# bjo5029/causal-vae

Hardware: AMD Instinct MI355X
Metric: training samples/sec on 128^3 vessel volumes (3D CausalVAE train step) (higher is better)
Workload: dtype bf16; 1 GPU; 3D vessel CausalVAE train step, 128^3 bf16 volumes (z-scored N(0,1)), batch 4/GPU, Adam lr 0.0001, ELBO = MSE-sum + 2000*MSE-sum(m) + KLD; global_batch=4, per_gpu_batch=4, parallelism=dp1, params=15346957

## Files before the change

### causal_vae_amd/csrc/conv_mfma.hip

```cpp
#include "common.h"

#ifdef CVAE_STAMP
#define CVAE_STAMP_SLOTS 32
#define CVAE_STAMP_WGS 8192
__device__ unsigned long long g_stamp[(size_t)CVAE_STAMP_WGS * CVAE_STAMP_SLOTS];
#define STAMP(i)                                                                                                         \
    do {                                                                                                                 \
        if (t == 0 && stamp_wg < CVAE_STAMP_WGS) g_stamp[(size_t)stamp_wg * CVAE_STAMP_SLOTS + (i)] = __builtin_readcyclecounter(); \
    } while (0)
#else
#define STAMP(i)
#endif

namespace {

CVAE_TUNABLE(BD_GS, 8);
CVAE_TUNABLE(APIPE, 3);
CVAE_TUNABLE(UPFULL_MIN_GRID, 2048);
CVAE_TUNABLE(UPFULL_MIN_WG, 512);
CVAE_TUNABLE(XPAIR_MIN_WGS, 2048);
CVAE_TUNABLE(XPAIR_2D_MIN_WGS, 512);
CVAE_TUNABLE(WG_TILES, 16);
CVAE_TUNABLE(WG_MIN_WG, 64);

// ... 1037 lines not shown
    float amx = 0.f;
    for (int64_t i = (((int64_t)blockIdx.x - tb.blk_start[ti]) * 256 + threadIdx.x) * 4; i < n; i += (int64_t)nb * 1024) {
        float v[4];
#pragma unroll
        for (int u = 0; u < 4; ++u) {
            const int64_t iu = i + u;
            const int e = (int)(iu % CH);
            int64_t rr = iu / CH;
            int cs, cl, tap;
            if (!for_up) { cs = (int)(rr % Cs); rr /= Cs; const int ch = (int)(rr % (Cl / CH)); tap = (int)(rr / (Cl / CH)); cl = ch * CH + e; }
            else { cl = (int)(rr % Cl); rr /= Cl; const int ch = (int)(rr % (Cs / CH)); tap = (int)(rr / (Cs / CH)); cs = ch * CH + e; }
            v[u] = w[((int64_t)cs * Cl + cl) * taps + tap];
            amx = fmaxf(amx, fabsf(v[u]));
            v[u] = __builtin_amdgcn_fmed3f(v[u] * mul, -CVAE_FP8_MAX, CVAE_FP8_MAX);
        }
        int c = __builtin_amdgcn_cvt_pk_fp8_f32(v[0], v[1], 0, false);
        c = __builtin_amdgcn_cvt_pk_fp8_f32(v[2], v[3], c, true);
        *(int*)(out + i) = c;
    }
    __shared__ float red[4];
    if (tb.amax[ti]) amax_publish_wg(tb.amax[ti], amx, blockIdx.x, red);
}

#define F8LAYER_MAX 16
struct F8LayerIdx { int in[F8LAYER_MAX], w[F8LAYER_MAX], out[F8LAYER_MAX]; int count; };
__global__ __launch_bounds__(1024) void fp8_scale_update_kernel(unsigned* __restrict__ amax, float* __restrict__ scale, float* __restrict__ inv_scale, int n, float headroom,
                                                                F8LayerIdx li, float* __restrict__ dscale, unsigned* __restrict__ ticket) {
    static_assert(CVAE_AMAX_SLOTS == 4096, "one uint4 per thread");
    __shared__ float red[16];
    __shared__ unsigned last;
    const int t = threadIdx.x, lane = t & 63, wave = t >> 6, i = blockIdx.x;
    uint4* a4 = (uint4*)amax + (size_t)i * (CVAE_AMAX_SLOTS / 4);
    const uint4 v = a4[t];
    a4[t] = make_uint4(0u, 0u, 0u, 0u);
    float a = fmaxf(fmaxf(__uint_as_float(v.x), __uint_as_float(v.y)), fmaxf(__uint_as_float(v.z), __uint_as_float(v.w)));
#pragma unroll
    for (int o = 32; o > 0; o >>= 1) a = fmaxf(a, __shfl_xor(a, o, 64));
    if (lane == 0) red[wave] = a;
    __syncthreads();
    if (t == 0) {
        float m = 0.f;
        for (int w_ = 0; w_ < 16; ++w_) m = fmaxf(m, red[w_]);
        if (m > 0.f) {
            const float s_ = headroom * m / CVAE_FP8_MAX;
            __hip_atomic_store(scale + i, s_, __ATOMIC_RELAXED, __HIP_MEMORY_SCOPE_AGENT);
            __hip_atomic_store(inv_scale + i, 1.f / s_, __ATOMIC_RELAXED, __HIP_MEMORY_SCOPE_AGENT);
        }
        asm volatile("s_waitcnt vmcnt(0)" ::: "memory");
        const unsigned got = __hip_atomic_fetch_add(ticket, 1u, __ATOMIC_RELAXED, __HIP_MEMORY_SCOPE_AGENT);
        last = (got == (unsigned)n - 1u) ? 1u : 0u;
    }
    __syncthreads();
    if (last && li.count > 0) {
        if (t < li.count) {
            const float si = __hip_atomic_load(scale + li.in[t], __ATOMIC_RELAXED, __HIP_MEMORY_SCOPE_AGENT);
            const float sw = __hip_atomic_load(scale + li.w[t], __ATOMIC_RELAXED, __HIP_MEMORY_SCOPE_AGENT);
            dscale[2 * t] = si * sw;
            dscale[2 * t + 1] = li.out[t] >= 0 ? 1.f / __hip_atomic_load(scale + li.out[t], __ATOMIC_RELAXED, __HIP_MEMORY_SCOPE_AGENT) : 0.f;
        }
    }
    if (last && t == 0) __hip_atomic_store(ticket, 0u, __ATOMIC_RELAXED, __HIP_MEMORY_SCOPE_AGENT);
}

__global__ __launch_bounds__(256) void absmax_kernel(const void* __restrict__ src, int dtype, int64_t n, unsigned* __restrict__ slots) {
    float amx = 0.f;
    for (int64_t i = blockIdx.x * (int64_t)blockDim.x + threadIdx.x; i < n; i += (int64_t)gridDim.x * blockDim.x)
        amx = fmaxf(amx, fabsf(dtype == CVAE_BF16 ? to_f32(((const bf16*)src)[i]) : ((const float*)src)[i]));
    __shared__ float red[4];
    amax_publish_wg(slots, amx, blockIdx.x, red);
}

#define PAIR_MAX 16
struct PairTable {
    const float* w[PAIR_MAX];
    void* down[PAIR_MAX];
    void* up[PAIR_MAX];
    int Cs[PAIR_MAX], Cl[PAIR_MAX], blk_start[PAIR_MAX + 1];
    int count;
    int f8dir[PAIR_MAX];
    fp8* f8out[PAIR_MAX];
    const float* inv_scale[PAIR_MAX];
    unsigned* amax[PAIR_MAX];
};
template <typename T, int TAPS>
__global__ __launch_bounds__(256) void pack_weight_pairs_kernel(PairTable tb) {
    constexpr int TT = 16, TSPLIT = TAPS / TT, TP = TT + 1;
    __shared__ float tile[16 * 17 * TP];
    int ti = 0;
    while (ti + 1 < tb.count && (int)blockIdx.x >= tb.blk_start[ti + 1]) ++ti;
    const int Cs = tb.Cs[ti], Cl = tb.Cl[ti];
    int blk = (int)blockIdx.x - tb.blk_start[ti];
    const int tq = blk % TSPLIT; blk /= TSPLIT;
    const int nclt = Cl / 16, ncst = Cs / 16;
    const int cst = blk / nclt, clt = blk % nclt, cs0 = cst * 16, cl0 = clt * 16;
    const float* w = tb.w[ti];
    const int f8dir = tb.f8dir[ti];
    float amx = 0.f;
#pragma unroll
    for (int it = 0; it < 4; ++it) {
        const int i = threadIdx.x + it * 256, f = i & 3, cl = (i >> 2) & 15, cs = i >> 6;
        const float4 v = *(const float4*)(w + ((size_t)(cs0 + cs) * Cl + cl0 + cl) * TAPS + tq * TT + 4 * f);
        float* d = tile + (cs * 17 + cl) * TP + 4 * f;
        d[0] = v.x; d[1] = v.y; d[2] = v.z; d[3] = v.w;
        amx = fmaxf(fmaxf(amx, fmaxf(fabsf(v.x), fabsf(v.y))), fmaxf(fabsf(v.z), fabsf(v.w)));
    }
    __syncthreads();
    T* od = (T*)tb.down[ti];
    T* ou = (T*)tb.up[ti];
    const float mul8 = f8dir ? tb.inv_scale[ti][0] : 1.f;
    const int tg = threadIdx.x >> 5, e0 = (threadIdx.x & 31) * 8, a = e0 >> 4, b0 = e0 & 15;
#pragma unroll
    for (int tl = tg; tl < TT; tl += 8) {
        const int tap = tq * TT + tl;
        __attribute__((aligned(16))) T vd[8], vu[8];
#pragma unroll
        for (int q = 0; q < 8; ++q) {
            vd[q] = from_f32<T>(tile[(a * 17 + b0 + q) * TP + tl]);
            vu[q] = from_f32<T>(tile[((b0 + q) * 17 + a) * TP + tl]);
        }
        T* pd = od + ((size_t)(tap * nclt + clt) * Cs + cs0 + a) * 16 + b0;
        T* pu = ou + ((size_t)(tap * ncst + cst) * Cl + cl0 + a) * 16 + b0;
        constexpr int NU = (8 * sizeof(T)) / 16;
        if (f8dir != 1) {
#pragma unroll
            for (int u = 0; u < NU; ++u) ((uint4*)pd)[u] = ((const uint4*)vd)[u];
        }
        if (f8dir != 2) {
#pragma unroll
            for (int u = 0; u < NU; ++u) ((uint4*)pu)[u] = ((const uint4*)vu)[u];
        }
        if (f8dir) {
            float v8[8];
#pragma unroll
            for (int q = 0; q < 8; ++q) v8[q] = f8dir == 1 ? tile[(a * 17 + b0 + q) * TP + tl] : tile[((b0 + q) * 17 + a) * TP + tl];
            fp8* p8 = f8dir == 1 ? tb.f8out[ti] + ((size_t)(tap * (Cl / 32) + (cl0 >> 5)) * Cs + cs0 + a) * 32 + (cl0 & 16) + b0
                                 : tb.f8out[ti] + ((size_t)(tap * (Cs / 32) + (cs0 >> 5)) * Cl + cl0 + a) * 32 + (cs0 & 16) + b0;
            *(uint2*)p8 = pack8_fp8(v8, mul8);
        }
    }
    if (f8dir && tb.amax[ti]) {
        __syncthreads();
        amax_publish_wg(tb.amax[ti], amx, blockIdx.x, tile);
    }
}

#define WG_MULTI_MAX 8
struct WgradEntry {
    const void* S; const void* L; float* ws; float* bias_ws;
    ConvGeom g;
    int n_split, cb, tg, bias_mode;
    int xb;
};
struct WgradTable { WgradEntry e[WG_MULTI_MAX]; int blk_start[WG_MULTI_MAX + 1]; int count; };

template <typename T, int ND>
__global__ __launch_bounds__(512, sizeof(T) == 2 ? 4 : 2) void conv_wgrad_kernel(WgradTable tb) {
    int ti = 0;
    while (ti + 1 < tb.count && (int)blockIdx.x >= tb.blk_start[ti + 1]) ++ti;
    const T* __restrict__ S = (const T*)tb.e[ti].S;
    const T* __restrict__ L = (const T*)tb.e[ti].L;
    float* __restrict__ ws = tb.e[ti].ws;
    float* __restrict__ bias_ws = tb.e[ti].bias_ws;
    const ConvGeom g = tb.e[ti].g;
    const int n_split = tb.e[ti].n_split, bias_mode = tb.e[ti].bias_mode, grid_y = tb.e[ti].cb;
    const int xb = (ND == 2) ? tb.e[ti].xb : 0;
    int lb = (int)blockIdx.x - tb.blk_start[ti];
    const int bx = lb % n_split; lb /= n_split;
    const int by = lb % grid_y, bz = lb / grid_y;
    using TL = Tile<ND, 128>;
    constexpr int NT = 512;
    constexpr int TD = TL::TD, TH = TL::TH, TW = TL::TW;
    constexpr int IW1 = 2 * TW + 2, IW = IW1 + (ND == 2 ? 2 : 0), IH = 2 * TH + 2;
    constexpr int SROW = 64 * sizeof(T), LROW = 32 * sizeof(T);
    constexpr int S_BYTES = 128 * SROW;
    constexpr int FB = 8 * sizeof(T);
    extern __shared__ __attribute__((aligned(16))) char smem[];
    char* s_lds = smem;
    char* l_lds = smem + S_BYTES;
    const int t = threadIdx.x, lane = t & 63, wave = t >> 6;
    const int cl_blocks = g.Cl / 32;
    const int cs0 = (by / cl_blocks) * 64, cl0 = (by % cl_blocks) * 32;
    const int kd = (ND == 3) ? bz : 0;
    const int kh = wave & 3, sg = wave >> 2;
    constexpr int LHALF = IW / 2, LPLANE = TD * IH * LHALF;
    auto s_byte = [](int m, int c) -> int { return m * SROW + ((((c >> 3) ^ (((m >> 1) & 1) << 2)) << 3) + (c & 7)) * (int)sizeof(T); };
    auto l_row = [](int line, int x) -> int { return (x & 1) * LPLANE + line * LHALF + (x >> 1); };
    const int tiles_per_b = g.tiles_d * g.tiles_h * g.tiles_w, total_tiles = (xb ? (g.B + 1) / 2 : g.B) * tiles_per_b;
#ifdef CVAE_STAMP
    const unsigned stamp_wg = blockIdx.x;
    if (t == 0 && stamp_wg < CVAE_STAMP_WGS) {
        g_stamp[(size_t)stamp_wg * CVAE_STAMP_SLOTS + 30] = wall_clock64();
        g_stamp[(size_t)stamp_wg * CVAE_STAMP_SLOTS + 29] = ((unsigned long long)__builtin_amdgcn_s_getreg(63508) << 32) | __builtin_amdgcn_s_getreg(63492);
    }
    int stamp_it = 0;
#endif
    STAMP(0);

    f32x16 acc[4];
#pragma unroll
    for (int k = 0; k < 4; ++k)
#pragma unroll
        for (int e = 0; e < 16; ++e) acc[k][e] = 0.f;

    const bool bias_s = bias_mode == 1 && (by % cl_blocks) == 0 && kd == 0;
    const bool bias_l = bias_mode == 2 && (by / cl_blocks) == 0 && (ND == 2 || kd == 1 || kd == 2);
    float bacc = 0.f;
    constexpr int SN = (128 * 8) / NT, LNPOS = TD * IH * IW, LN = (LNPOS * 4 + NT - 1) / NT;
    Piece<T> sp[SN], lp[LN];
    unsigned okmask = 0;
    const int s_sample = g.sd * g.sh * g.sw * g.Cs, l_sample = g.ld * g.lh * g.lw * g.Cl;
    auto load_tile = [&](int tile) {
        int tt = tile;
        const int tw_i = tt % g.tiles_w; tt /= g.tiles_w;
        const int th_i = tt % g.tiles_h; tt /= g.tiles_h;
        const int td_i = tt % g.tiles_d;
        const int b = (tt / g.tiles_d) * (1 + xb);
        const int o0d = td_i * TD, o0h = th_i * TH, o0w = tw_i * TW;
        const T* Sb = S + (size_t)b * s_sample + cs0;
        const T* Lb = L + (size_t)b * l_sample + cl0;
        const bool b1ok = b + 1 < g.B;
        okmask = 0;
        int tz = t;
        asm volatile("" : "+v"(tz));
#pragma unroll
        for (int i = 0; i < SN; ++i) {
            const int it = tz + i * NT, piece = it & 7, m = it >> 3;
            const int w = m % TW, hh = m / TW % TH, d = m / (TW * TH);
            const int sx = (xb && w >= TW / 2) ? 1 : 0;
            const int od = o0d + d, oh = o0h + hh, ow = o0w + w - sx * (TW / 2);
            const bool ok = (od < g.sd) & (oh < g.sh) & (ow < g.sw) & (!sx | b1ok);
            const unsigned off = ((min(od, g.sd - 1) * g.sh + min(oh, g.sh - 1)) * g.sw + min(ow, g.sw - 1)) * g.Cs + piece * 8 + ((sx && b1ok) ? (unsigned)s_sample : 0u);
            piece_load_raw<T>(sp[i], Sb + off);
            okmask |= (unsigned)ok << i;
        }
#pragma unroll
        for (int i = 0; i < LN; ++i) {
            const int it = tz + i * NT, piece = it & 3, pos = min(it >> 2, LNPOS - 1);
            const int x = pos % IW, y = pos / IW % IH, d = pos / (IW * IH);
            const int sx = (xb && x >= IW / 2) ? 1 : 0;
            const int lz = (ND == 3) ? 2 * (o0d + d) - 1 + kd : 0, ly = 2 * o0h - 1 + y, lx = 2 * o0w - 1 + x - sx * (IW / 2);
            const bool ok = (lz >= 0) & (lz < g.ld) & (ly >= 0) & (ly < g.lh) & (lx >= 0) & (lx < g.lw) & (!sx | b1ok) & (xb | (x < IW1));
            const unsigned off = ((min(max(lz, 0), g.ld - 1) * g.lh + min(max(ly, 0), g.lh - 1)) * g.lw + min(max(lx, 0), g.lw - 1)) * g.Cl + piece * 8 + ((sx && b1ok) ? (unsigned)l_sample : 0u);
            piece_load_raw<T>(lp[i], Lb + off);
            okmask |= (unsigned)ok << (SN + i);
        }
    };
    if (bx < total_tiles) load_tile(bx);
    for (int tile = bx; tile < total_tiles; tile += n_split) {
        __syncthreads();
#ifdef CVAE_STAMP
        if (stamp_it < 8) STAMP(2 + 3 * stamp_it);
#endif
        {
            int tz = t;
            asm volatile("" : "+v"(tz));
#pragma unroll
            for (int i = 0; i < SN; ++i) {
                const int it = tz + i * NT;
                piece_store_sel<T>(sp[i], (okmask >> i) & 1, s_lds + s_byte(it >> 3, (it & 7) * 8));
            }
#pragma unroll
            for (int i = 0; i < LN; ++i) {
                const int it = tz + i * NT, pos = it >> 2;
                if (it < LNPOS * 4) piece_store_sel<T>(lp[i], (okmask >> (SN + i)) & 1, l_lds + (l_row(pos / IW, pos % IW) * 4 + (it & 3)) * FB);
            }
        }
        __syncthreads();
#ifdef CVAE_STAMP
        if (stamp_it < 8) STAMP(3 + 3 * stamp_it);
#endif
        if (tile + n_split < total_tiles) load_tile(tile + n_split);
        if (bias_s) {
            const int c = t & 63, pg = t >> 6;
#pragma unroll 4
            for (int j = 0; j < 16; ++j) bacc += to_f32(*(const T*)(s_lds + s_byte(pg * 16 + j, c)));
        } else if (bias_l) {
            const int c = t & 31, pg = t >> 5;
#pragma unroll 4
            for (int j = 0; j < 32; ++j) {
                const int pp = pg + 16 * j;
                const int xx = pp % (2 * TW), yy = pp / (2 * TW) % (2 * TH), dd = pp / (4 * TW * TH);
                const int xs = xx + 1 + ((xb && xx >= TW) ? 2 : 0);
                bacc += to_f32(*(const T*)(l_lds + l_row(dd * IH + yy + 1, xs) * LROW + c * (int)sizeof(T)));
            }
        }
        if constexpr (sizeof(T) == 2) {
            const int gq = lane >> 4, i16 = lane & 15, q = i16 >> 2, p = i16 & 3;
            const int hk = gq >> 1, colblk = gq & 1;
            typedef __attribute__((address_space(3))) bf16x4 lds_bf16x4;
            const char* abase[2];
            const char* bbase[2];
#pragma unroll
            for (int jj = 0; jj < 2; ++jj) {
                const int r0 = 8 * hk + 4 * jj + q;
                abase[jj] = s_lds + s_byte(r0, sg * 32 + 16 * colblk + 4 * p);
                bbase[jj] = l_lds + l_row(2 * (r0 / TW) + kh, 2 * (r0 % TW) + ((xb && (r0 % TW) >= TW / 2) ? 2 : 0)) * LROW + (16 * colblk + 4 * p) * 2;
            }
#pragma unroll
            for (int c = 0; c < 8; ++c) {
                const int hh_c = (16 * c / TW) % TH, d_c = (16 * c) / (TW * TH);
                bf16x8 a;
#pragma unroll
                for (int jj = 0; jj < 2; ++jj) {
                    const bf16x4 v = __builtin_amdgcn_ds_read_tr16_b64_v4bf16((lds_bf16x4*)(abase[jj] + 16 * c * SROW));
                    a[4 * jj + 0] = v[0]; a[4 * jj + 1] = v[1]; a[4 * jj + 2] = v[2]; a[4 * jj + 3] = v[3];
                }
#pragma unroll
                for (int kw = 0; kw < 4; ++kw) {
                    bf16x8 bv;
#pragma unroll
                    for (int jj = 0; jj < 2; ++jj) {
                        const char* bp = bbase[jj] + (((kw & 1) * LPLANE + (d_c * IH + 2 * hh_c) * LHALF + (kw >> 1)) * LROW);
                        const bf16x4 v = __builtin_amdgcn_ds_read_tr16_b64_v4bf16((lds_bf16x4*)bp);
                        bv[4 * jj + 0] = v[0]; bv[4 * jj + 1] = v[1]; bv[4 * jj + 2] = v[2]; bv[4 * jj + 3] = v[3];
                    }
                    acc[kw] = __builtin_amdgcn_mfma_f32_32x32x16_bf16(a, bv, acc[kw], 0, 0, 0);
                }
            }
        } else {
            const int r = lane & 31, hk = lane >> 5;
#pragma unroll 1
            for (int mm = 0; mm < 128; mm += 2) {
                const int m = mm + hk;
                const int w = m % TW, hh = m / TW % TH, d = m / (TW * TH);
                const int line = d * IH + 2 * hh + kh;
                const float a = *(const float*)(s_lds + s_byte(m, sg * 32 + r));
#pragma unroll
                for (int kw = 0; kw < 4; ++kw) {
                    const float bv = *(const float*)(l_lds + l_row(line, 2 * w + kw + ((xb && w >= TW / 2) ? 2 : 0)) * LROW + r * 4);
                    acc[kw] = __builtin_amdgcn_mfma_f32_32x32x2f32(a, bv, acc[kw], 0, 0, 0);
                }
            }
        }
#ifdef CVAE_STAMP
        if (stamp_it < 8) STAMP(4 + 3 * stamp_it);
        ++stamp_it;
#endif
    }
    STAMP(26);
    if (bias_s || bias_l) {
        __syncthreads();
        float* red = (float*)s_lds;
        red[t] = bacc;
        __syncthreads();
        if (bias_s && t < 64) {
            float v = 0.f;
#pragma unroll
            for (int q = 0; q < 8; ++q) v += red[q * 64 + t];
            bias_ws[((size_t)(by / cl_blocks) * n_split + bx) * 64 + t] = v;
        }
        if (bias_l && t < 32) {
            float v = 0.f;
#pragma unroll
            for (int q = 0; q < 16; ++q) v += red[q * 32 + t];
            const int half = (ND == 3) ? kd - 1 : 0, nhalf = (ND == 3) ? 2 : 1;
            bias_ws[(((size_t)(by % cl_blocks) * nhalf + half) * n_split + bx) * 32 + t] = v;
        }
    }
    const int col = lane & 31, hq = lane >> 5;
    float* slab = ws + ((size_t)(bz * grid_y + by) * n_split + bx) * 32768;
#pragma unroll
    for (int e = 0; e < 16; ++e) {
        const int row = sg * 32 + (e & 3) + 8 * (e >> 2) + 4 * hq;
        *(float4*)(slab + ((kh * 64 + row) * 32 + col) * 4) = make_float4(acc[0][e], acc[1][e], acc[2][e], acc[3][e]);
    }
#ifdef CVAE_STAMP
    __builtin_amdgcn_s_waitcnt(0);
    STAMP(27);
    if (t == 0 && stamp_wg < CVAE_STAMP_WGS) g_stamp[(size_t)stamp_wg * CVAE_STAMP_SLOTS + 31] = wall_clock64();
#endif
}

struct WgradReduceEntry {
    const float* ws; float* dW; const float* bias_ws; float* dbias;
    int Cs, Cl, n_split, cb, dw_blocks, bias_n, bias_rows, bias_width;
};
struct WgradReduceTable { WgradReduceEntry e[WG_MULTI_MAX]; int blk_start[WG_MULTI_MAX + 1]; int count, taps; };
__global__ __launch_bounds__(256) void wgrad_reduce_kernel(WgradReduceTable tb) {
    int ti = 0;
    while (ti + 1 < tb.count && (int)blockIdx.x >= tb.blk_start[ti + 1]) ++ti;
    const float* __restrict__ ws = tb.e[ti].ws;
    float* __restrict__ dW = tb.e[ti].dW;
    const float* __restrict__ bias_ws = tb.e[ti].bias_ws;
    float* __restrict__ dbias = tb.e[ti].dbias;
    const int Cl = tb.e[ti].Cl, taps = tb.taps, n_split = tb.e[ti].n_split, cb = tb.e[ti].cb, dw_blocks = tb.e[ti].dw_blocks;
    const int bias_n = tb.e[ti].bias_n, bias_rows = tb.e[ti].bias_rows, bias_width = tb.e[ti].bias_width;
    const int lbx = (int)blockIdx.x - tb.blk_start[ti];
    __shared__ float4 part[4][64];
    if (lbx >= dw_blocks) {
        __shared__ float bred[4][64];
        const int ch = (lbx - dw_blocks) * 64 + (threadIdx.x & 63), q = threadIdx.x >> 6;
        float v = 0.f;
        if (ch < bias_n) {
            const float* base = bias_ws + (size_t)(ch / bias_width) * bias_rows * bias_width + (ch % bias_width);
            for (int r = q; r < bias_rows; r += 4) v += base[(size_t)r * bias_width];
        }
        bred[q][threadIdx.x & 63] = v;
        __syncthreads();
        if (q == 0 && ch < bias_n) dbias[ch] = bred[0][threadIdx.x] + bred[1][threadIdx.x] + bred[2][threadIdx.x] + bred[3][threadIdx.x];
        return;
    }
    const int cl_blocks = Cl / 32;
    int bi = lbx;
    const int rowpair = bi % 32; bi /= 32;
    const int kh = bi % 4; bi /= 4;
    const int grp = bi;
    const int kd = grp / cb, blk = grp % cb;
    const int lane64 = threadIdx.x & 63, q = threadIdx.x >> 6;
    const int row = rowpair * 2 + (lane64 >> 5), col = lane64 & 31;
    const float* base = ws + (size_t)grp * n_split * 32768 + ((kh * 64 + row) * 32 + col) * 4;
    float4 a = make_float4(0.f, 0.f, 0.f, 0.f);
    constexpr int U = 8;
    for (int x0 = q; x0 < n_split; x0 += 4 * U) {
        float4 v[U];
#pragma unroll
        for (int u = 0; u < U; ++u) v[u] = *(const float4*)(base + (size_t)min(x0 + 4 * u, n_split - 1) * 32768);
#pragma unroll
        for (int u = 0; u < U; ++u)
            if (x0 + 4 * u < n_split) { a.x += v[u].x; a.y += v[u].y; a.z += v[u].z; a.w += v[u].w; }
    }
    part[q][lane64] = a;
    __syncthreads();
    if (q == 0) {
        const float4 b = part[1][lane64], c = part[2][lane64], d = part[3][lane64];
        a.x += b.x + c.x + d.x; a.y += b.y + c.y + d.y; a.z += b.z + c.z + d.z; a.w += b.w + c.w + d.w;
        const int cs = (blk / cl_blocks) * 64 + row, cl = (blk % cl_blocks) * 32 + col;
        *(float4*)(dW + ((size_t)cs * Cl + cl) * taps + kd * 16 + kh * 4) = a;
    }
}

#define WGRAD_MAX_WG 512
template <typename T, int ND> constexpr size_t wgrad_lds_bytes() {
    using TL = Tile<ND, 128>;
    return (size_t)128 * 64 * sizeof(T) + (size_t)TL::TD * (2 * TL::TH + 2) * (2 * TL::TW + 2 + (ND == 2 ? 2 : 0)) * 32 * sizeof(T);
}
template <typename T, int ND>
int plan_wgrad(const void* S, const void* L, float* ws, float* dW, float* dbias, int bias_mode, ConvGeom g, WgradEntry* me, WgradReduceEntry* re, int* main_blocks,
               int* reduce_blocks, long long n_split_req = 0) {
    using TL = Tile<ND, 128>;
    g.tiles_d = (g.sd + TL::TD - 1) / TL::TD; g.tiles_h = (g.sh + TL::TH - 1) / TL::TH; g.tiles_w = (g.sw + TL::TW - 1) / TL::TW;
    const int xb = (ND == 2 && g.sw <= TL::TW / 2 && g.B >= 2) ? 1 : 0;
    const long long total_tiles = (long long)(xb ? (g.B + 1) / 2 : g.B) * g.tiles_d * g.tiles_h * g.tiles_w;
    const int cb = (g.Cs / 64) * (g.Cl / 32), tg = (ND == 3) ? 4 : 1;
    long long n_split = WGRAD_MAX_WG / ((long long)cb * tg);
    long long floor_split = 256 / ((long long)cb * tg);
    if (floor_split > total_tiles) floor_split = total_tiles;
    long long by_tiles = total_tiles / 4;
    if (by_tiles < floor_split) by_tiles = floor_split;
    if (n_split > by_tiles) n_split = by_tiles;
    {
        long long req = (total_tiles + WG_TILES - 1) / WG_TILES;
        const long long groups = (long long)cb * tg;
        if (req * groups < WG_MIN_WG) req = (WG_MIN_WG + groups - 1) / groups;
        if (req < n_split) n_split = req;
    }
    if (n_split_req > 0 && n_split_req < n_split) n_split = n_split_req;
    if (n_split < 1) n_split = 1;
    if (n_split > total_tiles) n_split = total_tiles;
    if ((long long)cb * tg * n_split > (1 << 24)) return CVAE_E_BADSHAPE;
    const long long wgs = (long long)cb * tg * n_split;
    float* bias_ws = ws + (size_t)(wgs > WGRAD_MAX_WG ? wgs : WGRAD_MAX_WG) * 32768;
    if (!dbias) bias_mode = 0;
    *me = WgradEntry{S, L, ws, bias_ws, g, (int)n_split, cb, tg, bias_mode, xb};
    *main_blocks = (int)wgs;
    const int dw_blocks = cb * tg * 4 * 32;
    const int bias_n = bias_mode == 1 ? g.Cs : (bias_mode == 2 ? g.Cl : 0), bias_width = bias_mode == 1 ? 64 : 32;
    const int bias_rows = (int)n_split * ((bias_mode == 2 && ND == 3) ? 2 : 1);
    *re = WgradReduceEntry{ws, dW, bias_ws, dbias, g.Cs, g.Cl, (int)n_split, cb, dw_blocks, bias_n, bias_rows, bias_width};
    *reduce_blocks = dw_blocks + (bias_n + 63) / 64;
    return CVAE_OK;
}
template <typename T, int ND>
int launch_wgrad_tables(WgradTable& mt, WgradReduceTable& rt, hipStream_t stream) {
    constexpr size_t LDS = wgrad_lds_bytes<T, ND>();
    static_assert(LDS <= 160 * 1024, "LDS tile exceeds the 160 KiB of a CDNA4 CU");
    auto kern = conv_wgrad_kernel<T, ND>;
    static bool attr_set = false;
    if (!attr_set) {
        if (hipFuncSetAttribute((const void*)kern, hipFuncAttributeMaxDynamicSharedMemorySize, (int)LDS) != hipSuccess) return CVAE_E_LAUNCH;
        attr_set = true;
    }
    rt.taps = (ND == 3) ? 64 : 16;
    hipLaunchKernelGGL(kern, dim3((unsigned)mt.blk_start[mt.count]), dim3(512), LDS, stream, mt);
    CVAE_CHECK_LAUNCH();
    hipLaunchKernelGGL(wgrad_reduce_kernel, dim3((unsigned)rt.blk_start[rt.count]), dim3(256), 0, stream, rt);
    CVAE_CHECK_LAUNCH();
    return CVAE_OK;
}
template <typename T, int ND>
int launch_wgrad(const void* S, const void* L, float* ws, float* dW, float* dbias, int bias_mode, ConvGeom g, hipStream_t stream) {
    WgradTable mt;
    WgradReduceTable rt;
    int mb, rb;
    const int rc = plan_wgrad<T, ND>(S, L, ws, dW, dbias, bias_mode, g, &mt.e[0], &rt.e[0], &mb, &rb);
    if (rc != CVAE_OK) return rc;
    mt.count = rt.count = 1;
    mt.blk_start[0] = rt.blk_start[0] = 0;
    mt.blk_start[1] = mb; rt.blk_start[1] = rb;
    return launch_wgrad_tables<T, ND>(mt, rt, stream);
}

bool geom_ok(int64_t B, int64_t sd, int64_t sh, int64_t sw, int64_t Cs, int64_t ld, int64_t lh, int64_t lw, int64_t Cl, int nd) {
    if (nd != 2 && nd != 3) return false;
    if (B < 0 || sd <= 0 || sh <= 0 || sw <= 0 || Cs <= 0 || ld <= 0 || lh <= 0 || lw <= 0 || Cl <= 0) return false;
    if (B > 65535 || sd > 32767 || sh > 32767 || sw > 32767 || ld > 65535 || lh > 65535 || lw > 65535) return false;
    if (nd == 2 && (sd != 1 || ld != 1)) return false;
    if (sd * sh * sw * Cs >= (int64_t(1) << 31) || ld * lh * lw * Cl >= (int64_t(1) << 31)) return false;
    auto pair_ok = [](int64_t s, int64_t l) { return s == l / 2; };
    if (nd == 3 && !pair_ok(sd, ld)) return false;
    return pair_ok(sh, lh) && pair_ok(sw, lw) && lh >= 2 && lw >= 2 && (nd == 2 || ld >= 2);
}

}

int cvae_conv_down_c1(const void* L, int l_dtype, const float* w, const float* bias, const void* mask, void* S, int64_t B, int64_t sd, int64_t sh, int64_t sw,
                      int64_t Cs, int64_t ld, int64_t lh, int64_t lw, int nd, int dtype, int act, hipStream_t stream, F8Side f8 = F8Side{nullptr, nullptr, nullptr});
int cvae_conv_up_c1(const void* S, const float* w, const float* bias, const void* mask, void* L, int64_t B, int64_t sd, int64_t sh, int64_t sw,
                    int64_t Cs, int64_t ld, int64_t lh, int64_t lw, int nd, int dtype, int act, hipStream_t stream, long long walk_units = 0);
int cvae_conv_up_c1_fp8in_impl(const void* S8, const float* w, const float* bias, void* L, float in_scale, int64_t B, int64_t sd, int64_t sh, int64_t sw, int64_t Cs, int act,
                               hipStream_t stream);
size_t cvae_conv_wgrad_c1_workspace_bytes(int64_t Cs, int nd);
int cvae_conv_wgrad_c1(const void* S, const void* L, int l_dtype, float* dW, float* dbias, float* dbias_l, void* workspace, size_t workspace_bytes, int64_t B, int64_t sd, int64_t sh,
                       int64_t sw, int64_t Cs, int64_t ld, int64_t lh, int64_t lw, int nd, int dtype, hipStream_t stream);

#ifdef CVAE_STAMP
extern "C" int cvae_debug_stamps(unsigned long long* host, size_t count) {
    if (count > (size_t)CVAE_STAMP_WGS * CVAE_STAMP_SLOTS) return CVAE_E_BADSHAPE;
    return hipMemcpyFromSymbol(host, HIP_SYMBOL(g_stamp), count * sizeof(unsigned long long)) == hipSuccess ? CVAE_OK : CVAE_E_LAUNCH;
}
#endif

extern "C" int cvae_conv_pack_weight(const float* w, void* packed, int64_t Cs, int64_t Cl, int nd, int for_up, int dtype, void* stream) {
    if ((nd != 2 && nd != 3) || Cs <= 0 || Cl <= 0) return CVAE_E_BADSHAPE;
    if ((!for_up && Cl % 16) || (for_up && (Cs % 16 || Cl % 32))) return CVAE_E_UNSUPPORTED;
    if (!w || !packed) return CVAE_E_NULLPTR;
    const int taps = (nd == 3) ? 64 : 16;
    const int64_t n = Cs * Cl * taps;
    if (dtype == CVAE_BF16) hipLaunchKernelGGL(pack_weight_kernel<bf16>, dim3(cvae_grid_1d(n, 256)), dim3(256), 0, (hipStream_t)stream, w, (bf16*)packed, (int)Cs, (int)Cl, taps, for_up);
    else if (dtype == CVAE_F32) hipLaunchKernelGGL(pack_weight_kernel<float>, dim3(cvae_grid_1d(n, 256)), dim3(256), 0, (hipStream_t)stream, w, (float*)packed, (int)Cs, (int)Cl, taps, for_up);
    else return CVAE_E_DTYPE;
    CVAE_CHECK_LAUNCH();
    return CVAE_OK;
}

static bool fp8_pack_ok(int64_t Cs, int64_t Cl, int for_up) { return for_up ? (Cs % 32 == 0 && Cl % 32 == 0 && Cl > 1) : (Cl % 32 == 0 && Cs % 64 == 0); }
extern "C" int cvae_conv_pack_weight_pairs(const float* const* w, void* const* packed_down, void* const* packed_up, const int64_t* Cs, const int64_t* Cl,
                                           const int* f8dir, void* const* f8out, const float* const* inv_scale_dev, void* const* amax_slots,
                                           int count, int nd, int dtype, void* stream) {
    if ((nd != 2 && nd != 3) || count < 0) return CVAE_E_BADSHAPE;
    if (count == 0) return CVAE_OK;
    if (!w || !packed_down || !packed_up || !Cs || !Cl) return CVAE_E_NULLPTR;
    if (dtype != CVAE_BF16 && dtype != CVAE_F32) return CVAE_E_DTYPE;
    const int tsplit = (nd == 3) ? 4 : 1;
    for (int c0 = 0; c0 < count; c0 += PAIR_MAX) {
        PairTable tb;
        const int cnt = (count - c0 < PAIR_MAX) ? count - c0 : PAIR_MAX;
        long long blocks = 0;
        for (int i = 0; i < cnt; ++i) {
            const int64_t cs = Cs[c0 + i], cl = Cl[c0 + i];
            if (cs <= 0 || cl <= 0) return CVAE_E_BADSHAPE;
            if (cs % 16 || cl % 16) return CVAE_E_UNSUPPORTED;
            const int fd = f8dir ? f8dir[c0 + i] : 0;
            if (fd < 0 || fd > 2) return CVAE_E_BADSHAPE;
            if (fd) {
                if (dtype != CVAE_BF16) return CVAE_E_DTYPE;
                if (!fp8_pack_ok(cs, cl, fd == 2)) return CVAE_E_UNSUPPORTED;
                if (!f8out || !f8out[c0 + i] || !inv_scale_dev || !inv_scale_dev[c0 + i]) return CVAE_E_NULLPTR;
            }
            if (!w[c0 + i] || (fd != 1 && !packed_down[c0 + i]) || (fd != 2 && !packed_up[c0 + i])) return CVAE_E_NULLPTR;
            tb.w[i] = w[c0 + i]; tb.down[i] = packed_down[c0 + i]; tb.up[i] = packed_up[c0 + i]; tb.Cs[i] = (int)cs; tb.Cl[i] = (int)cl;
            tb.f8dir[i] = fd; tb.f8out[i] = fd ? (fp8*)f8out[c0 + i] : nullptr; tb.inv_scale[i] = fd ? inv_scale_dev[c0 + i] : nullptr;
            tb.amax[i] = (fd && amax_slots) ? (unsigned*)amax_slots[c0 + i] : nullptr;
            tb.blk_start[i] = (int)blocks;
            blocks += (cs / 16) * (cl / 16) * tsplit;
            if (blocks > (1 << 30)) return CVAE_E_BADSHAPE;
        }
        tb.blk_start[cnt] = (int)blocks;
        tb.count = cnt;
        const dim3 grid((unsigned)blocks);
        hipStream_t st = (hipStream_t)stream;
        if (dtype == CVAE_BF16) {
            if (nd == 3) hipLaunchKernelGGL((pack_weight_pairs_kernel<bf16, 64>), grid, dim3(256), 0, st, tb);
            else hipLaunchKernelGGL((pack_weight_pairs_kernel<bf16, 16>), grid, dim3(256), 0, st, tb);
        } else {
            if (nd == 3) hipLaunchKernelGGL((pack_weight_pairs_kernel<float, 64>), grid, dim3(256), 0, st, tb);
            else hipLaunchKernelGGL((pack_weight_pairs_kernel<float, 16>), grid, dim3(256), 0, st, tb);
        }
        CVAE_CHECK_LAUNCH();
    }
    return CVAE_OK;
}

#define GEOM_INIT() ConvGeom g{(int)B, (int)sd, (int)sh, (int)sw, (int)Cs, (int)ld, (int)lh, (int)lw, (int)Cl, 0, 0, 0}

extern "C" size_t cvae_conv_data_workspace_bytes(int64_t B, int64_t sd, int64_t sh, int64_t sw, int64_t Cs,
                                                  int64_t ld, int64_t lh, int64_t lw, int64_t Cl, int nd, int for_up) {
    if (!geom_ok(B, sd, sh, sw, Cs, ld, lh, lw, Cl, nd) || B == 0 || Cl == 1) return 0;
    GEOM_INIT();
    const bool wide = !for_up || Cl % 64 == 0;
    if (for_up ? (Cs % 16 || Cl % 32) : (Cl % 16 || Cs % 64)) return 0;
    return with_nd(nd, [&](auto n) { return with_bool(for_up != 0, [&](auto up) { return with_bool(wide, [&](auto wd) {
        return data_workspace_bytes<decltype(n)::value, decltype(up)::value, decltype(wd)::value>(g);
    }); }); });
}

static bool bits_ok(int64_t Cout) { return Cout % 32 == 0; }
extern "C" int cvae_conv_down(const void* L, const void* w, const float* bias, const void* mask, const void* mask_bits, void* S, void* relu_bits_out,
                              int64_t B, int64_t sd, int64_t sh, int64_t sw, int64_t Cs,
                              int64_t ld, int64_t lh, int64_t lw, int64_t Cl, int nd, int dtype, int act,
                              void* workspace, size_t workspace_bytes, int xpair, void* stream) {
    if (xpair < -1 || xpair > 1 || (mask && mask_bits)) return CVAE_E_BADSHAPE;
    if ((mask_bits || relu_bits_out) && !bits_ok(Cs)) return CVAE_E_UNSUPPORTED;
    if (Cl == 1 && mask_bits && !(dtype == CVAE_BF16)) return CVAE_E_UNSUPPORTED;
    F8Side side{nullptr, nullptr, nullptr};
    side.mask_bits = (const unsigned*)mask_bits; side.bits_out = (unsigned*)relu_bits_out;
    UpVariant var;
    var.xpair = xpair;
    if (!geom_ok(B, sd, sh, sw, Cs, ld, lh, lw, Cl, nd)) return CVAE_E_BADSHAPE;
    if (dtype != CVAE_F32 && dtype != CVAE_BF16) return CVAE_E_DTYPE;
    if (B == 0) return CVAE_OK;
    if (!L || !w || !S) return CVAE_E_NULLPTR;
    hipStream_t st = (hipStream_t)stream;
    if (Cl == 1) return cvae_conv_down_c1(L, dtype, (const float*)w, bias, mask, S, B, sd, sh, sw, Cs, ld, lh, lw, nd, dtype, act, st, side);
    if (Cl % 16 || Cs % 64) return CVAE_E_UNSUPPORTED;
    GEOM_INIT();
    const ConvArgs a{L, w, bias, mask, S, g, act, workspace, workspace_bytes, st, 1.f, 1.f, side, var};
    return with_dtype(dtype, [&](auto t) { return with_nd(nd, [&](auto n) { return dispatch_conv<decltype(t), decltype(n)::value, false, true>(a); }); });
}
extern "C" int cvae_conv_image_supported(const void* L, int64_t lw, int l_dtype, int dtype) {
    if (l_dtype == dtype) return 1;
    if (!(dtype == CVAE_BF16 && l_dtype == CVAE_F32)) return 0;
    return lw % 4 == 0 && lw >= 4 && (((uintptr_t)L) & 15) == 0;
}
extern "C" int cvae_conv_down_image(const void* L, int l_dtype, const float* w, const float* bias, const void* mask, void* S,
                                    int64_t B, int64_t sd, int64_t sh, int64_t sw, int64_t Cs, int64_t ld, int64_t lh, int64_t lw, int nd, int dtype, int act, void* stream) {
    if (!geom_ok(B, sd, sh, sw, Cs, ld, lh, lw, 1, nd)) return CVAE_E_BADSHAPE;
// ... 298 lines not shown
```

Measured before the change: 5128 samples/s.

## Pair two 512-thread wgrad teams per 1024-thread workgroup with in-LDS accumulator merge

For bf16 weight-gradient convolution, each workgroup now runs 1024 threads as two independent 512-thread teams. Each team has its own LDS tile buffer and processes alternate tiles of the split. At the end, the teams merge their MFMA accumulators through shared memory before a single write to the workspace. The number of splits is halved, so the workspace and the reduce kernel handle half as many partial slices, at the cost of extra barriers across 1024 threads, doubled LDS per workgroup and possible occupancy or register pressure changes.

```diff
diff --git a/causal_vae_amd/csrc/conv_mfma.hip b/causal_vae_amd/csrc/conv_mfma.hip
--- a/causal_vae_amd/csrc/conv_mfma.hip
+++ b/causal_vae_amd/csrc/conv_mfma.hip
@@ -1213,9 +1213,13 @@
     int xb;
 };
 struct WgradTable { WgradEntry e[WG_MULTI_MAX]; int blk_start[WG_MULTI_MAX + 1]; int count; };
+template <typename T, int ND> constexpr size_t wgrad_tile_bytes() {
+    using TL = Tile<ND, 128>;
+    return (size_t)128 * 64 * sizeof(T) + (size_t)TL::TD * (2 * TL::TH + 2) * (2 * TL::TW + 2 + (ND == 2 ? 2 : 0)) * 32 * sizeof(T);
+}
 
 template <typename T, int ND>
-__global__ __launch_bounds__(512, sizeof(T) == 2 ? 4 : 2) void conv_wgrad_kernel(WgradTable tb) {
+__global__ __launch_bounds__(sizeof(T) == 2 ? 1024 : 512, sizeof(T) == 2 ? 4 : 2) void conv_wgrad_kernel(WgradTable tb) {
     int ti = 0;
     while (ti + 1 < tb.count && (int)blockIdx.x >= tb.blk_start[ti + 1]) ++ti;
     const T* __restrict__ S = (const T*)tb.e[ti].S;
@@ -1229,16 +1233,19 @@
     const int bx = lb % n_split; lb /= n_split;
     const int by = lb % grid_y, bz = lb / grid_y;
     using TL = Tile<ND, 128>;
+    constexpr bool PAIR = sizeof(T) == 2;
     constexpr int NT = 512;
     constexpr int TD = TL::TD, TH = TL::TH, TW = TL::TW;
     constexpr int IW1 = 2 * TW + 2, IW = IW1 + (ND == 2 ? 2 : 0), IH = 2 * TH + 2;
     constexpr int SROW = 64 * sizeof(T), LROW = 32 * sizeof(T);
-    constexpr int S_BYTES = 128 * SROW;
+    constexpr int S_BYTES = 128 * SROW, TILE_BYTES = S_BYTES + TD * IH * IW * LROW;
+    static_assert(TILE_BYTES == (int)wgrad_tile_bytes<T, ND>() && TILE_BYTES % 16 == 0, "the launch sizes the LDS by wgrad_tile_bytes");
     constexpr int FB = 8 * sizeof(T);
     extern __shared__ __attribute__((aligned(16))) char smem[];
-    char* s_lds = smem;
-    char* l_lds = smem + S_BYTES;
-    const int t = threadIdx.x, lane = t & 63, wave = t >> 6;
+    const int half = PAIR ? (int)threadIdx.x >> 9 : 0;
+    const int t = threadIdx.x & (NT - 1), lane = t & 63, wave = t >> 6;
+    char* s_lds = smem + half * TILE_BYTES;
+    char* l_lds = s_lds + S_BYTES;
     const int cl_blocks = g.Cl / 32;
     const int cs0 = (by / cl_blocks) * 64, cl0 = (by % cl_blocks) * 32;
     const int kd = (ND == 3) ? bz : 0;
@@ -1248,7 +1255,7 @@
     auto l_row = [](int line, int x) -> int { return (x & 1) * LPLANE + line * LHALF + (x >> 1); };
     const int tiles_per_b = g.tiles_d * g.tiles_h * g.tiles_w, total_tiles = (xb ? (g.B + 1) / 2 : g.B) * tiles_per_b;
 #ifdef CVAE_STAMP
-    const unsigned stamp_wg = blockIdx.x;
+    const unsigned stamp_wg = half ? CVAE_STAMP_WGS : blockIdx.x;
     if (t == 0 && stamp_wg < CVAE_STAMP_WGS) {
         g_stamp[(size_t)stamp_wg * CVAE_STAMP_SLOTS + 30] = wall_clock64();
         g_stamp[(size_t)stamp_wg * CVAE_STAMP_SLOTS + 29] = ((unsigned long long)__builtin_amdgcn_s_getreg(63508) << 32) | __builtin_amdgcn_s_getreg(63492);
@@ -1306,13 +1313,17 @@
             okmask |= (unsigned)ok << (SN + i);
         }
     };
-    if (bx < total_tiles) load_tile(bx);
-    for (int tile = bx; tile < total_tiles; tile += n_split) {
+    const int step = PAIR ? 2 * n_split : n_split;
+    const int slab_tiles = (total_tiles - bx + n_split - 1) / n_split, rounds = PAIR ? (slab_tiles + 1) / 2 : slab_tiles;
+    int tile = bx + half * n_split;
+    if (tile < total_tiles) load_tile(tile);
+    for (int rd = 0; rd < rounds; ++rd, tile += step) {
+        const bool active = tile < total_tiles;
         __syncthreads();
 #ifdef CVAE_STAMP
         if (stamp_it < 8) STAMP(2 + 3 * stamp_it);
 #endif
-        {
+        if (active) {
             int tz = t;
             asm volatile("" : "+v"(tz));
 #pragma unroll
@@ -1330,7 +1341,8 @@
 #ifdef CVAE_STAMP
         if (stamp_it < 8) STAMP(3 + 3 * stamp_it);
 #endif
-        if (tile + n_split < total_tiles) load_tile(tile + n_split);
+        if (!active) continue;
+        if (tile + step < total_tiles) load_tile(tile + step);
         if (bias_s) {
             const int c = t & 63, pg = t >> 6;
 #pragma unroll 4
@@ -1401,21 +1413,38 @@
     STAMP(26);
     if (bias_s || bias_l) {
         __syncthreads();
-        float* red = (float*)s_lds;
-        red[t] = bacc;
+        constexpr int TEAMS = PAIR ? 2 : 1;
+        const int tx = threadIdx.x;
+        float* red = (float*)smem;
+        red[tx] = bacc;
         __syncthreads();
-        if (bias_s && t < 64) {
+        if (bias_s && tx < 64) {
             float v = 0.f;
 #pragma unroll
-            for (int q = 0; q < 8; ++q) v += red[q * 64 + t];
-            bias_ws[((size_t)(by / cl_blocks) * n_split + bx) * 64 + t] = v;
-        }
-        if (bias_l && t < 32) {
+            for (int q = 0; q < 8 * TEAMS; ++q) v += red[q * 64 + tx];
+            bias_ws[((size_t)(by / cl_blocks) * n_split + bx) * 64 + tx] = v;
+        }
+        if (bias_l && tx < 32) {
             float v = 0.f;
 #pragma unroll
-            for (int q = 0; q < 16; ++q) v += red[q * 32 + t];
-            const int half = (ND == 3) ? kd - 1 : 0, nhalf = (ND == 3) ? 2 : 1;
-            bias_ws[(((size_t)(by % cl_blocks) * nhalf + half) * n_split + bx) * 32 + t] = v;
+            for (int q = 0; q < 16 * TEAMS; ++q) v += red[q * 32 + tx];
+            const int par = (ND == 3) ? kd - 1 : 0, npar = (ND == 3) ? 2 : 1;
+            bias_ws[(((size_t)(by % cl_blocks) * npar + par) * n_split + bx) * 32 + tx] = v;
+        }
+    }
+    if constexpr (PAIR) {
+        __syncthreads();
+        float4* mg = (float4*)smem + wave * (16 * 64) + lane;
+        if (half == 1) {
+#pragma unroll
+            for (int e = 0; e < 16; ++e) mg[e * 64] = make_float4(acc[0][e], acc[1][e], acc[2][e], acc[3][e]);
+        }
+        __syncthreads();
+        if (half == 1) return;
+#pragma unroll
+        for (int e = 0; e < 16; ++e) {
+            const float4 v = mg[e * 64];
+            acc[0][e] += v.x; acc[1][e] += v.y; acc[2][e] += v.z; acc[3][e] += v.w;
         }
     }
     const int col = lane & 31, hq = lane >> 5;
@@ -1492,8 +1521,7 @@
 
 #define WGRAD_MAX_WG 512
 template <typename T, int ND> constexpr size_t wgrad_lds_bytes() {
-    using TL = Tile<ND, 128>;
-    return (size_t)128 * 64 * sizeof(T) + (size_t)TL::TD * (2 * TL::TH + 2) * (2 * TL::TW + 2 + (ND == 2 ? 2 : 0)) * 32 * sizeof(T);
+    return sizeof(T) == 2 ? (2 * wgrad_tile_bytes<T, ND>() > 131072 ? 2 * wgrad_tile_bytes<T, ND>() : 131072) : wgrad_tile_bytes<T, ND>();
 }
 template <typename T, int ND>
 int plan_wgrad(const void* S, const void* L, float* ws, float* dW, float* dbias, int bias_mode, ConvGeom g, WgradEntry* me, WgradReduceEntry* re, int* main_blocks,
@@ -1516,6 +1544,7 @@
         if (req < n_split) n_split = req;
     }
     if (n_split_req > 0 && n_split_req < n_split) n_split = n_split_req;
+    if (sizeof(T) == 2) n_split = (n_split + 1) / 2;
     if (n_split < 1) n_split = 1;
     if (n_split > total_tiles) n_split = total_tiles;
     if ((long long)cb * tg * n_split > (1 << 24)) return CVAE_E_BADSHAPE;
@@ -1542,7 +1571,7 @@
         attr_set = true;
     }
     rt.taps = (ND == 3) ? 64 : 16;
-    hipLaunchKernelGGL(kern, dim3((unsigned)mt.blk_start[mt.count]), dim3(512), LDS, stream, mt);
+    hipLaunchKernelGGL(kern, dim3((unsigned)mt.blk_start[mt.count]), dim3(sizeof(T) == 2 ? 1024 : 512), LDS, stream, mt);
     CVAE_CHECK_LAUNCH();
     hipLaunchKernelGGL(wgrad_reduce_kernel, dim3((unsigned)rt.blk_start[rt.count]), dim3(256), 0, stream, rt);
     CVAE_CHECK_LAUNCH();
```

Result: slower. 5036 samples/s (-1.8%).
